# YannDubs/disentangling-vae

Measured on AMD Instinct MI355X. Metric: images/sec (whole node) at 64x64x3, btcvae loss, higher is better.
Workload: dtype f32; 1 GPU; btcvae_celeba (BASELINE.json configs[3]): Burgess VAE 64x64x3, btcvae loss, z=10, tensor handed to _train_iteration B=1024 global (1024 per GPU), Adam lr 0.0005, n_data=202599, fwd+loss+bwd+Adam; batch_per_gpu=1024, global_batch=1024, parallelism=dp1

## Files before the change

### disentangling-vae_amd/csrc/linear_grouped.hip

```cpp
#include "common.h"

namespace dvae {

struct FcwProb {
  const float* x; const float* dy; float* dw; float* db;
  int M, N, K, tile0, tk, flags;
};
struct FcwTable { FcwProb p[DVAE_FCW_MAX]; int n; };

template <int KP>
__global__ __launch_bounds__(256) void k_fcw_grouped(const FcwTable t) {
  extern __shared__ __attribute__((aligned(16))) float fcg_lds[];
  constexpr int S = KP / 8;
  constexpr int NB = KP / 32;
  constexpr int ROWS = KP + 8;
  float* As = fcg_lds;
  float* Bs = fcg_lds + ROWS * 32;
  const int tid = threadIdx.x, lane = tid & 63;
  const int wv = __builtin_amdgcn_readfirstlane(tid >> 6);
  const int i = lane & 31, h = lane >> 5;
  const int bid = blockIdx.x;

  const float* x = t.p[0].x; const float* dy = t.p[0].dy; float* dw = t.p[0].dw; float* db = t.p[0].db;
  int M = t.p[0].M, N = t.p[0].N, K = t.p[0].K, tile0 = 0, tk = t.p[0].tk, flags = t.p[0].flags;
#pragma unroll
  for (int q = 1; q < DVAE_FCW_MAX; ++q) {
    if (q < t.n && bid >= t.p[q].tile0) {
      x = t.p[q].x; dy = t.p[q].dy; dw = t.p[q].dw; db = t.p[q].db;
      M = t.p[q].M; N = t.p[q].N; K = t.p[q].K; tile0 = t.p[q].tile0; tk = t.p[q].tk; flags = t.p[q].flags;
    }
  }
  const int tile = bid - tile0;
  const int n0 = (tile / tk) * 32, k0 = (tile % tk) * 32;
  const int j4 = (tid & 7) * 4;
  const bool vecA = flags & 1, vecB = flags & 2;

  f32x16 acc[4];
#pragma unroll
  for (int q = 0; q < 4; ++q)
#pragma unroll
    for (int e = 0; e < 16; ++e) acc[q][e] = 0.f;
  float rs = 0.f;
  f32x4 ra[NB], rb[NB];
  int mload = 0;
  auto load = [&](int m0) {
    mload = m0;
#pragma unroll
    for (int p = 0; p < NB; ++p) {
      const int m = m0 + (tid >> 3) + 32 * p;
      const long mm = m < M ? m : M - 1;
      const float* pa = dy + mm * N;
      const float* pb = x + mm * K;
      if (vecA) {
        ra[p] = *reinterpret_cast<const f32x4*>(pa + (n0 + j4 < N ? n0 + j4 : 0));
      } else {
#pragma unroll
        for (int u = 0; u < 4; ++u) ra[p][u] = pa[n0 + j4 + u < N ? n0 + j4 + u : 0];
      }
      if (vecB) {
        rb[p] = *reinterpret_cast<const f32x4*>(pb + (k0 + j4 < K ? k0 + j4 : 0));
      } else {
#pragma unroll
        for (int u = 0; u < 4; ++u) rb[p][u] = pb[k0 + j4 + u < K ? k0 + j4 + u : 0];
      }
    }
  };
  const int kap0 = (2 * wv + h) * S;
  const float* ap = As + (kap0 + 2 * wv + h) * 32 + i;
  const float* bp = Bs + (kap0 + 2 * wv + h) * 32 + i;
  load(0);
  for (int m0 = 0; m0 < M; m0 += KP) {
    if (m0) __syncthreads();
#pragma unroll
    for (int p = 0; p < NB; ++p) {
      const int kap = (tid >> 3) + 32 * p;
      const bool in = mload + kap < M;
      f32x4 va, vb;
#pragma unroll
      for (int u = 0; u < 4; ++u) {
        va[u] = (in && n0 + j4 + u < N) ? ra[p][u] : 0.f;
        vb[u] = (in && k0 + j4 + u < K) ? rb[p][u] : 0.f;
      }
      *reinterpret_cast<f32x4*>(As + (kap + kap / S) * 32 + j4) = va;
      *reinterpret_cast<f32x4*>(Bs + (kap + kap / S) * 32 + j4) = vb;
    }
    __syncthreads();
    if (m0 + KP < M) load(m0 + KP);
#pragma unroll
    for (int tt = 0; tt < S; tt += 4) {
      float av[4], bv[4];
#pragma unroll
      for (int u = 0; u < 4; ++u) { av[u] = ap[(tt + u) * 32]; bv[u] = bp[(tt + u) * 32]; }
#pragma unroll
      for (int u = 0; u < 4; ++u) {
        acc[u] = __builtin_amdgcn_mfma_f32_32x32x2f32(av[u], bv[u], acc[u], 0, 0, 0);
        rs += av[u];
      }
    }
  }
  const f32x16 accs = (acc[0] + acc[1]) + (acc[2] + acc[3]);
  __syncthreads();
  float* red = fcg_lds;
  float* rsum = fcg_lds + 4 * 16 * 64;
#pragma unroll
  for (int e = 0; e < 16; ++e) red[(wv * 16 + e) * 64 + lane] = accs[e];
  rs += __shfl_xor(rs, 32, 64);
  if (h == 0) rsum[wv * 32 + i] = rs;
  __syncthreads();
  const int col = k0 + i;
#pragma unroll
  for (int u = 0; u < 4; ++u) {
    const int e = 4 * wv + u;
    const int row = n0 + (e & 3) + 8 * (e >> 2) + 4 * h;
    const float v = (red[(0 * 16 + e) * 64 + lane] + red[(1 * 16 + e) * 64 + lane]) +
                    (red[(2 * 16 + e) * 64 + lane] + red[(3 * 16 + e) * 64 + lane]);
    if (row < N && col < K) dw[(long)row * K + col] = v;
  }
  if (db && k0 == 0 && wv == 0 && h == 0 && n0 + i < N)
    db[n0 + i] = (rsum[i] + rsum[32 + i]) + (rsum[64 + i] + rsum[96 + i]);
}

template <int KP>
static void launch_fcw_grouped_t(const FcwTable& t, int tiles, hipStream_t s) {
  const size_t lds = sizeof(float) * 2 * (KP + 8) * 32;
  static DeviceOnce attr;
  if (attr.first()) {
    (void)hipFuncSetAttribute((const void*)k_fcw_grouped<KP>, hipFuncAttributeMaxDynamicSharedMemorySize, (int)lds);
  }
  hipLaunchKernelGGL((k_fcw_grouped<KP>), dim3(tiles), dim3(256), lds, s, t);
}

int launch_linear_wgrad_grouped(const dvae_linear_wgrad_desc* d, int n, hipStream_t s) {
  FcwTable t;
  memset(&t, 0, sizeof(t));
  t.n = n;
  int tiles = 0, maxM = 0;
  for (int q = 0; q < n; ++q) {
    FcwProb& p = t.p[q];
    p.x = d[q].x; p.dy = d[q].dy; p.dw = d[q].dw; p.db = d[q].db;
    p.M = d[q].M; p.N = d[q].N; p.K = d[q].K;
    p.tile0 = tiles;
    p.tk = (p.K + 31) / 32;
    p.flags = ((p.N % 4 == 0 && ((uintptr_t)p.dy & 15) == 0) ? 1 : 0) | ((p.K % 4 == 0 && ((uintptr_t)p.x & 15) == 0) ? 2 : 0);
    tiles += p.tk * ((p.N + 31) / 32);
    if (p.M > maxM) maxM = p.M;
  }
  if (maxM <= 64) launch_fcw_grouped_t<64>(t, tiles, s);
  else if (maxM <= 128) launch_fcw_grouped_t<128>(t, tiles, s);
  else launch_fcw_grouped_t<256>(t, tiles, s);
  DVAE_CHECK_LAUNCH();
  return 0;
}

}
```

Baseline: 996,300 images/s.

## Load FC weight-grad operands directly into MFMA registers via buffer loads, bypassing LDS

Rewrites the grouped linear weight-gradient kernel so each wave loads its MFMA operands straight from global memory with raw buffer loads. Row-blocks are assigned round-robin across the four waves and double-buffered in registers, which drops the LDS staging and the per-chunk barriers. Out-of-range row blocks are neutralised by zeroing the buffer descriptor's record count. LDS is now used only for the final cross-wave reduction. In exchange, loads become scalar per lane instead of 16-byte vector loads, and the code depends on compiler scheduling barriers to keep loads overlapped with MFMAs.

Result: no change. 1.002 million images/s (median of 6 runs) (+0.6%).

```diff
diff --git a/disentangling-vae_amd/csrc/fcw_body.h b/disentangling-vae_amd/csrc/fcw_body.h
--- /dev/null
+++ b/disentangling-vae_amd/csrc/fcw_body.h
@@ -0,0 +1,146 @@
+#pragma once
+#include "common.h"
+
+namespace dvae {
+
+struct FcwProb {
+  const float* x; const float* dy; float* dw; float* db;
+  int M, N, K, tile0, tk;
+};
+struct FcwTable { FcwProb p[DVAE_FCW_MAX]; int n; };
+
+constexpr int FCW_RED_FLOATS = 4 * 16 * 64 + 4 * 32;
+
+typedef float fcw_f32x2 __attribute__((ext_vector_type(2)));
+
+__device__ __forceinline__ __amdgpu_buffer_rsrc_t fcw_rsrc(const float* p, int records = -1) {
+  return __builtin_amdgcn_make_buffer_rsrc(const_cast<float*>(p), 0, records, 0x00020000);
+}
+__device__ __forceinline__ float fcw_ld(__amdgpu_buffer_rsrc_t r, unsigned voff, unsigned soff) {
+  const unsigned v = __builtin_amdgcn_raw_buffer_load_b32(r, (int)voff, (int)soff, 0);
+  return __builtin_bit_cast(float, v);
+}
+
+template <int KP>
+__device__ __forceinline__ void fcw_contract(const float* __restrict__ x, const float* __restrict__ dy, int M, int N, int K,
+                                             int n0, int k0, int wv, int lane, f32x16 (&acc)[4], fcw_f32x2& rs) {
+  constexpr int BR = KP >= 128 ? 32 : 16;
+  constexpr int U = BR / 2;
+  const int i = lane & 31, h = lane >> 5;
+  const unsigned ca = n0 + i < N ? n0 + i : N - 1, cb = k0 + i < K ? k0 + i : K - 1;
+  const unsigned pa = 8u * (unsigned)N, pb = 8u * (unsigned)K;
+  const int nfull = M / BR;
+  const int nk = nfull > wv ? (nfull - wv + 3) / 4 : 0;
+  const unsigned va = 4u * ((unsigned)h * N + ca), vb = 4u * ((unsigned)h * K + cb);
+  float a0[U], b0[U], a1[U], b1[U];
+  auto base = [&](const float* p, int ld, int k) {
+    int live;
+    asm("s_ashr_i32 %0, %1, 31" : "=s"(live) : "s"(__builtin_amdgcn_readfirstlane(k - nk)) : "scc");
+    const int row = ((wv + 4 * k) * BR) & live;
+    return fcw_rsrc(p + (long)row * ld, live);
+  };
+  auto fill = [&](float (&a)[U], float (&b)[U], int k) {
+    const __amdgpu_buffer_rsrc_t ra = base(dy, N, k), rb = base(x, K, k);
+#pragma unroll
+    for (int u = 0; u < U; ++u) { a[u] = fcw_ld(ra, va, u * pa); b[u] = fcw_ld(rb, vb, u * pb); }
+  };
+  auto stage = [&](float (&a)[U], float (&b)[U], int kn) {
+    const __amdgpu_buffer_rsrc_t ra = base(dy, N, kn), rb = base(x, K, kn);
+#pragma unroll
+    for (int u = 0; u < U; u += 2) {
+      acc[u & 3] = __builtin_amdgcn_mfma_f32_32x32x2f32(a[u], b[u], acc[u & 3], 0, 0, 0);
+      acc[(u + 1) & 3] = __builtin_amdgcn_mfma_f32_32x32x2f32(a[u + 1], b[u + 1], acc[(u + 1) & 3], 0, 0, 0);
+      rs += fcw_f32x2{a[u], a[u + 1]};
+      a[u] = fcw_ld(ra, va, u * pa);
+      b[u] = fcw_ld(rb, vb, u * pb);
+      a[u + 1] = fcw_ld(ra, va, (u + 1) * pa);
+      b[u + 1] = fcw_ld(rb, vb, (u + 1) * pb);
+      __builtin_amdgcn_sched_barrier(0);
+    }
+  };
+  fill(a0, b0, 0);
+  fill(a1, b1, 1);
+  int k = 0;
+  for (; k + 1 < nk; k += 2) {
+    stage(a0, b0, k + 2);
+    stage(a1, b1, k + 3);
+  }
+  if (k < nk) {
+#pragma unroll
+    for (int u = 0; u < U; u += 2) {
+      acc[u & 3] = __builtin_amdgcn_mfma_f32_32x32x2f32(a0[u], b0[u], acc[u & 3], 0, 0, 0);
+      acc[(u + 1) & 3] = __builtin_amdgcn_mfma_f32_32x32x2f32(a0[u + 1], b0[u + 1], acc[(u + 1) & 3], 0, 0, 0);
+      rs += fcw_f32x2{a0[u], a0[u + 1]};
+    }
+  }
+  const int mt = nfull * BR;
+  if (mt < M && (nfull & 3) == wv) {
+    const __amdgpu_buffer_rsrc_t ra = fcw_rsrc(dy + (long)mt * N), rb = fcw_rsrc(x + (long)mt * K);
+    const int rem = M - mt;
+#pragma unroll
+    for (int u = 0; u < U; ++u) {
+      const int r = 2 * u + h < rem ? 2 * u + h : rem - 1;
+      a0[u] = fcw_ld(ra, 4u * ((unsigned)r * N + ca), 0);
+      b0[u] = fcw_ld(rb, 4u * ((unsigned)r * K + cb), 0);
+    }
+#pragma unroll
+    for (int u = 0; u < U; u += 2) {
+      const bool in0 = 2 * u + h < rem, in1 = 2 * u + 2 + h < rem;
+      const float av0 = in0 ? a0[u] : 0.f, bv0 = in0 ? b0[u] : 0.f, av1 = in1 ? a0[u + 1] : 0.f, bv1 = in1 ? b0[u + 1] : 0.f;
+      acc[u & 3] = __builtin_amdgcn_mfma_f32_32x32x2f32(av0, bv0, acc[u & 3], 0, 0, 0);
+      acc[(u + 1) & 3] = __builtin_amdgcn_mfma_f32_32x32x2f32(av1, bv1, acc[(u + 1) & 3], 0, 0, 0);
+      rs += fcw_f32x2{av0, av1};
+    }
+  }
+}
+
+template <int KP>
+__device__ __forceinline__ void fcw_grouped_body(const FcwTable& t, float* lds) {
+  const int tid = threadIdx.x, lane = tid & 63;
+  const int wv = __builtin_amdgcn_readfirstlane(tid >> 6);
+  const int i = lane & 31, h = lane >> 5;
+  const int bid = blockIdx.x;
+
+  const float* x = t.p[0].x; const float* dy = t.p[0].dy; float* dw = t.p[0].dw; float* db = t.p[0].db;
+  int M = t.p[0].M, N = t.p[0].N, K = t.p[0].K, tile0 = 0, tk = t.p[0].tk;
+#pragma unroll
+  for (int q = 1; q < DVAE_FCW_MAX; ++q) {
+    if (q < t.n && bid >= t.p[q].tile0) {
+      x = t.p[q].x; dy = t.p[q].dy; dw = t.p[q].dw; db = t.p[q].db;
+      M = t.p[q].M; N = t.p[q].N; K = t.p[q].K; tile0 = t.p[q].tile0; tk = t.p[q].tk;
+    }
+  }
+  const int tile = bid - tile0;
+  const int n0 = (tile / tk) * 32, k0 = (tile % tk) * 32;
+
+  f32x16 acc[4];
+#pragma unroll
+  for (int q = 0; q < 4; ++q)
+#pragma unroll
+    for (int e = 0; e < 16; ++e) acc[q][e] = 0.f;
+  fcw_f32x2 rs2 = {0.f, 0.f};
+  fcw_contract<KP>(x, dy, M, N, K, n0, k0, wv, lane, acc, rs2);
+
+  const f32x16 accs = (acc[0] + acc[1]) + (acc[2] + acc[3]);
+  float* red = lds;
+  float* rsum = lds + 4 * 16 * 64;
+#pragma unroll
+  for (int e = 0; e < 16; ++e) red[(wv * 16 + e) * 64 + lane] = accs[e];
+  float rs = rs2[0] + rs2[1];
+  rs += __shfl_xor(rs, 32, 64);
+  if (h == 0) rsum[wv * 32 + i] = rs;
+  __syncthreads();
+  const int col = k0 + i;
+#pragma unroll
+  for (int u = 0; u < 4; ++u) {
+    const int e = 4 * wv + u;
+    const int row = n0 + (e & 3) + 8 * (e >> 2) + 4 * h;
+    const float v = (red[(0 * 16 + e) * 64 + lane] + red[(1 * 16 + e) * 64 + lane]) +
+                    (red[(2 * 16 + e) * 64 + lane] + red[(3 * 16 + e) * 64 + lane]);
+    if (row < N && col < K) dw[(long)row * K + col] = v;
+  }
+  if (db && k0 == 0 && wv == 0 && h == 0 && n0 + i < N)
+    db[n0 + i] = (rsum[i] + rsum[32 + i]) + (rsum[64 + i] + rsum[96 + i]);
+}
+
+}
diff --git a/disentangling-vae_amd/csrc/linear_grouped.hip b/disentangling-vae_amd/csrc/linear_grouped.hip
--- a/disentangling-vae_amd/csrc/linear_grouped.hip
+++ b/disentangling-vae_amd/csrc/linear_grouped.hip
@@ -1,128 +1,17 @@
 #include "common.h"
+#include "fcw_body.h"
 
 namespace dvae {
-
-struct FcwProb {
-  const float* x; const float* dy; float* dw; float* db;
-  int M, N, K, tile0, tk, flags;
-};
-struct FcwTable { FcwProb p[DVAE_FCW_MAX]; int n; };
 
 template <int KP>
 __global__ __launch_bounds__(256) void k_fcw_grouped(const FcwTable t) {
   extern __shared__ __attribute__((aligned(16))) float fcg_lds[];
-  constexpr int S = KP / 8;
-  constexpr int NB = KP / 32;
-  constexpr int ROWS = KP + 8;
-  float* As = fcg_lds;
-  float* Bs = fcg_lds + ROWS * 32;
-  const int tid = threadIdx.x, lane = tid & 63;
-  const int wv = __builtin_amdgcn_readfirstlane(tid >> 6);
-  const int i = lane & 31, h = lane >> 5;
-  const int bid = blockIdx.x;
-
-  const float* x = t.p[0].x; const float* dy = t.p[0].dy; float* dw = t.p[0].dw; float* db = t.p[0].db;
-  int M = t.p[0].M, N = t.p[0].N, K = t.p[0].K, tile0 = 0, tk = t.p[0].tk, flags = t.p[0].flags;
-#pragma unroll
-  for (int q = 1; q < DVAE_FCW_MAX; ++q) {
-    if (q < t.n && bid >= t.p[q].tile0) {
-      x = t.p[q].x; dy = t.p[q].dy; dw = t.p[q].dw; db = t.p[q].db;
-      M = t.p[q].M; N = t.p[q].N; K = t.p[q].K; tile0 = t.p[q].tile0; tk = t.p[q].tk; flags = t.p[q].flags;
-    }
-  }
-  const int tile = bid - tile0;
-  const int n0 = (tile / tk) * 32, k0 = (tile % tk) * 32;
-  const int j4 = (tid & 7) * 4;
-  const bool vecA = flags & 1, vecB = flags & 2;
-
-  f32x16 acc[4];
-#pragma unroll
-  for (int q = 0; q < 4; ++q)
-#pragma unroll
-    for (int e = 0; e < 16; ++e) acc[q][e] = 0.f;
-  float rs = 0.f;
-  f32x4 ra[NB], rb[NB];
-  int mload = 0;
-  auto load = [&](int m0) {
-    mload = m0;
-#pragma unroll
-    for (int p = 0; p < NB; ++p) {
-      const int m = m0 + (tid >> 3) + 32 * p;
-      const long mm = m < M ? m : M - 1;
-      const float* pa = dy + mm * N;
-      const float* pb = x + mm * K;
-      if (vecA) {
-        ra[p] = *reinterpret_cast<const f32x4*>(pa + (n0 + j4 < N ? n0 + j4 : 0));
-      } else {
-#pragma unroll
-        for (int u = 0; u < 4; ++u) ra[p][u] = pa[n0 + j4 + u < N ? n0 + j4 + u : 0];
-      }
-      if (vecB) {
-        rb[p] = *reinterpret_cast<const f32x4*>(pb + (k0 + j4 < K ? k0 + j4 : 0));
-      } else {
-#pragma unroll
-        for (int u = 0; u < 4; ++u) rb[p][u] = pb[k0 + j4 + u < K ? k0 + j4 + u : 0];
-      }
-    }
-  };
-  const int kap0 = (2 * wv + h) * S;
-  const float* ap = As + (kap0 + 2 * wv + h) * 32 + i;
-  const float* bp = Bs + (kap0 + 2 * wv + h) * 32 + i;
-  load(0);
-  for (int m0 = 0; m0 < M; m0 += KP) {
-    if (m0) __syncthreads();
-#pragma unroll
-    for (int p = 0; p < NB; ++p) {
-      const int kap = (tid >> 3) + 32 * p;
-      const bool in = mload + kap < M;
-      f32x4 va, vb;
-#pragma unroll
-      for (int u = 0; u < 4; ++u) {
-        va[u] = (in && n0 + j4 + u < N) ? ra[p][u] : 0.f;
-        vb[u] = (in && k0 + j4 + u < K) ? rb[p][u] : 0.f;
-      }
-      *reinterpret_cast<f32x4*>(As + (kap + kap / S) * 32 + j4) = va;
-      *reinterpret_cast<f32x4*>(Bs + (kap + kap / S) * 32 + j4) = vb;
-    }
-    __syncthreads();
-    if (m0 + KP < M) load(m0 + KP);
-#pragma unroll
-    for (int tt = 0; tt < S; tt += 4) {
-      float av[4], bv[4];
-#pragma unroll
-      for (int u = 0; u < 4; ++u) { av[u] = ap[(tt + u) * 32]; bv[u] = bp[(tt + u) * 32]; }
-#pragma unroll
-      for (int u = 0; u < 4; ++u) {
-        acc[u] = __builtin_amdgcn_mfma_f32_32x32x2f32(av[u], bv[u], acc[u], 0, 0, 0);
-        rs += av[u];
-      }
-    }
-  }
-  const f32x16 accs = (acc[0] + acc[1]) + (acc[2] + acc[3]);
-  __syncthreads();
-  float* red = fcg_lds;
-  float* rsum = fcg_lds + 4 * 16 * 64;
-#pragma unroll
-  for (int e = 0; e < 16; ++e) red[(wv * 16 + e) * 64 + lane] = accs[e];
-  rs += __shfl_xor(rs, 32, 64);
-  if (h == 0) rsum[wv * 32 + i] = rs;
-  __syncthreads();
-  const int col = k0 + i;
-#pragma unroll
-  for (int u = 0; u < 4; ++u) {
-    const int e = 4 * wv + u;
-    const int row = n0 + (e & 3) + 8 * (e >> 2) + 4 * h;
-    const float v = (red[(0 * 16 + e) * 64 + lane] + red[(1 * 16 + e) * 64 + lane]) +
-                    (red[(2 * 16 + e) * 64 + lane] + red[(3 * 16 + e) * 64 + lane]);
-    if (row < N && col < K) dw[(long)row * K + col] = v;
-  }
-  if (db && k0 == 0 && wv == 0 && h == 0 && n0 + i < N)
-    db[n0 + i] = (rsum[i] + rsum[32 + i]) + (rsum[64 + i] + rsum[96 + i]);
+  fcw_grouped_body<KP>(t, fcg_lds);
 }
 
 template <int KP>
 static void launch_fcw_grouped_t(const FcwTable& t, int tiles, hipStream_t s) {
-  const size_t lds = sizeof(float) * 2 * (KP + 8) * 32;
+  const size_t lds = sizeof(float) * FCW_RED_FLOATS;
   static DeviceOnce attr;
   if (attr.first()) {
     (void)hipFuncSetAttribute((const void*)k_fcw_grouped<KP>, hipFuncAttributeMaxDynamicSharedMemorySize, (int)lds);
@@ -141,7 +30,6 @@
     p.M = d[q].M; p.N = d[q].N; p.K = d[q].K;
     p.tile0 = tiles;
     p.tk = (p.K + 31) / 32;
-    p.flags = ((p.N % 4 == 0 && ((uintptr_t)p.dy & 15) == 0) ? 1 : 0) | ((p.K % 4 == 0 && ((uintptr_t)p.x & 15) == 0) ? 2 : 0);
     tiles += p.tk * ((p.N + 31) / 32);
     if (p.M > maxM) maxM = p.M;
   }
```
